# eloialonso/diamond

Hardware: AMD Instinct MI355X
Metric: imagined frames/sec (64x64, 3 denoise steps, batch 256) (higher is better)
Workload: dtype f32 via split-f16 MFMA (world-model convs (3x3 stride 1 / 2, 1x1): fp32 operands split into 2 x fp16 pieces, 3 x v_mfma_f32_*_f16 per product, fp32 accumulate (fp32-class, 22-bit operands); attention core, linears: exact fp32 v_mfma_f32_16x16x4_f32; actor-critic encoder forward, dgrad and weight-gra

## Files before the change

### diamond_amd/csrc/dmd_linear.hip

```cpp
#include "dmd_common.h"

#define LIN_DEPTH 4

__device__ __forceinline__ f32x4 lin_frag(const float* rowp, size_t ks, int k, int K) {
  f32x4 v;
#pragma unroll
  for (int t = 0; t < 4; ++t) {
    const int kk = k + t;
    const float x = rowp[(size_t)(kk < K ? kk : K - 1) * ks];
    v[t] = kk < K ? x : 0.f;
  }
  return v;
}

template <bool SPLITK, bool TRANS>
__device__ __forceinline__ void linear_mfma_body(const dmd_linear_params& p) {
  __shared__ f32x4 part[SPLITK ? 3 : 1][4][64];
  const int lane = threadIdx.x & 63, wave = threadIdx.x >> 6;
  const int i = lane & 15, kg = lane >> 4;
  const int m0 = SPLITK ? blockIdx.x * 32 : blockIdx.x * 64 + (wave >> 1) * 32;
  const int n0 = SPLITK ? blockIdx.y * 32 : blockIdx.y * 64 + (wave & 1) * 32;
  const int Kp = TRANS ? (p.K + 15) & ~15 : p.K;
  const int kq = SPLITK ? Kp >> 2 : Kp;
  const int kbase = SPLITK ? wave * kq : 0;
  const int nsteps = kq >> 4;
  f32x4 acc[2][2];
#pragma unroll
  for (int a = 0; a < 2; ++a)
#pragma unroll
    for (int b = 0; b < 2; ++b) acc[a][b] = (f32x4){0.f, 0.f, 0.f, 0.f};

  const size_t a_rs = TRANS && p.trans_a ? 1 : (size_t)p.lda, a_ks = TRANS && p.trans_a ? (size_t)p.lda : 1;
  const size_t w_rs = TRANS && p.trans_w ? 1 : (size_t)p.ldw, w_ks = TRANS && p.trans_w ? (size_t)p.ldw : 1;
  const float* arow[2];
  const float* wrow[2];
#pragma unroll
  for (int b = 0; b < 2; ++b) {
    int m = m0 + 16 * b + i;
    m = m < p.M ? m : p.M - 1;
    int n = n0 + 16 * b + i;
    n = n < p.N ? n : p.N - 1;
    if (TRANS) {
      arow[b] = p.A + (size_t)m * a_rs;
      wrow[b] = p.W + (size_t)n * w_rs;
    } else {
      arow[b] = p.A + (size_t)m * p.lda + kbase + 4 * kg;
      wrow[b] = p.W + (size_t)n * p.ldw + kbase + 4 * kg;
    }
  }
  const int kl = kbase + 4 * kg;
  f32x4 af[LIN_DEPTH][2], wf[LIN_DEPTH][2];
#pragma unroll
  for (int d = 0; d < LIN_DEPTH; ++d) {
    const int ks = (d < nsteps ? d : nsteps - 1) * 16;
#pragma unroll
    for (int b = 0; b < 2; ++b) {
      if (TRANS) {
        af[d][b] = lin_frag(arow[b], a_ks, kl + ks, p.K);
        wf[d][b] = lin_frag(wrow[b], w_ks, kl + ks, p.K);
      } else {
        af[d][b] = *(const f32x4*)(arow[b] + ks);
        wf[d][b] = *(const f32x4*)(wrow[b] + ks);
      }
    }
  }
  for (int s0 = 0; s0 < nsteps; s0 += LIN_DEPTH) {
#pragma unroll
    for (int d = 0; d < LIN_DEPTH; ++d) {
      if (s0 + d < nsteps) {
#pragma unroll
        for (int nb = 0; nb < 2; ++nb)
#pragma unroll
          for (int mb = 0; mb < 2; ++mb)
#pragma unroll
            for (int t = 0; t < 4; ++t)
              acc[nb][mb] = __builtin_amdgcn_mfma_f32_16x16x4f32(wf[d][nb][t], af[d][mb][t], acc[nb][mb], 0, 0, 0);
        const int sn = s0 + d + LIN_DEPTH;
        const int ks = (sn < nsteps ? sn : nsteps - 1) * 16;
#pragma unroll
        for (int b = 0; b < 2; ++b) {
          if (TRANS) {
            af[d][b] = lin_frag(arow[b], a_ks, kl + ks, p.K);
            wf[d][b] = lin_frag(wrow[b], w_ks, kl + ks, p.K);
          } else {
            af[d][b] = *(const f32x4*)(arow[b] + ks);
            wf[d][b] = *(const f32x4*)(wrow[b] + ks);
          }
        }
      }
    }
  }
  if (SPLITK) {
    if (wave) {
#pragma unroll
      for (int nb = 0; nb < 2; ++nb)
#pragma unroll
        for (int mb = 0; mb < 2; ++mb) part[wave - 1][nb * 2 + mb][lane] = acc[nb][mb];
    }
    __syncthreads();
    if (wave) return;
#pragma unroll
    for (int w = 0; w < 3; ++w)
#pragma unroll
      for (int nb = 0; nb < 2; ++nb)
#pragma unroll
        for (int mb = 0; mb < 2; ++mb) acc[nb][mb] += part[w][nb * 2 + mb][lane];
  }
#pragma unroll
  for (int nb = 0; nb < 2; ++nb)
#pragma unroll
    for (int mb = 0; mb < 2; ++mb) {
      const int m = m0 + 16 * mb + i;
      const int n = n0 + 16 * nb + 4 * kg;
      if (m >= p.M) continue;
#pragma unroll
      for (int r = 0; r < 4; ++r) {
        if (n + r >= p.N) continue;
        float v = acc[nb][mb][r];
        if (p.bias) v += p.bias[n + r];
        float* c = p.C + (size_t)m * p.ldc + n + r;
        if (p.accumulate) v += *c;
        if (p.silu) v = dmd_silu(v);
        *c = v;
      }
    }
}

template <bool SPLITK>
__global__ __launch_bounds__(256) void linear_mfma_kernel(const dmd_linear_params p) {
  linear_mfma_body<SPLITK, false>(p);
}

template <bool SPLITK>
__global__ __launch_bounds__(256) void linear_mfma_t_kernel(const dmd_linear_params p) {
  linear_mfma_body<SPLITK, true>(p);
}

extern "C" int dmd_linear(const dmd_linear_params* p, dmd_stream_t stream) {
  DMD_CHECK_ARG(p && p->A && p->W && p->C, "linear: null");
  DMD_CHECK_ARG(p->M > 0 && p->N > 0 && p->K > 0, "linear: bad M/N/K %d %d %d", p->M, p->N, p->K);
  DMD_CHECK_ARG((p->trans_a | p->trans_w | 1) == 1, "linear: trans_a / trans_w are 0 or 1");
  const bool trans = p->trans_a || p->trans_w || p->K % 16 != 0 || p->lda % 4 != 0 || p->ldw % 4 != 0;
  const int Kp = (p->K + 15) / 16 * 16;
  const bool splitk = Kp >= 512 && Kp % 64 == 0;
  const dim3 grid = splitk ? dim3((p->M + 31) / 32, (p->N + 31) / 32) : dim3((p->M + 63) / 64, (p->N + 63) / 64);
  if (trans) {
    if (splitk)
      hipLaunchKernelGGL(linear_mfma_t_kernel<true>, grid, dim3(256), 0, (hipStream_t)stream, *p);
    else
      hipLaunchKernelGGL(linear_mfma_t_kernel<false>, grid, dim3(256), 0, (hipStream_t)stream, *p);
  } else if (splitk)
    hipLaunchKernelGGL(linear_mfma_kernel<true>, grid, dim3(256), 0, (hipStream_t)stream, *p);
  else
    hipLaunchKernelGGL(linear_mfma_kernel<false>, grid, dim3(256), 0, (hipStream_t)stream, *p);
  DMD_LAUNCH_CHECK();
  return 0;
}
```

### diamond_amd/native.py

```python
from __future__ import annotations

import ctypes as C
import os
from typing import Optional

import torch
from torch import Tensor

_HERE = os.path.dirname(os.path.abspath(__file__))
LIB_PATH = os.environ.get("DIAMOND_LIB", os.path.join(_HERE, "libdiamond_hip.so"))

PROLOGUE_NONE, PROLOGUE_NORM_SILU, PROLOGUE_NORM = 0, 1, 2
PRECISION_F32, PRECISION_F16X2 = 0, 1
GN_GROUP = 32


class NativeLibraryMissing(RuntimeError):
    pass


class Norm(C.Structure):
    _fields_ = [("stats", C.c_void_p), ("stat_tiles", C.c_int32), ("mul_plus_one", C.c_int32), ("mul", C.c_void_p),
                ("add", C.c_void_p), ("mul_stride", C.c_int64), ("add_stride", C.c_int64)]


class ConvSrc(C.Structure):
    _fields_ = [("x", C.c_void_p), ("C", C.c_int32), ("prologue", C.c_int32), ("norm", Norm)]


class ConvParams(C.Structure):
    _fields_ = [("N", C.c_int32), ("H", C.c_int32), ("W", C.c_int32), ("Cout", C.c_int32), ("CoutPad", C.c_int32),
                ("taps", C.c_int32), ("stride", C.c_int32), ("upsample", C.c_int32), ("nsrc", C.c_int32),
                ("src", ConvSrc * 2), ("w", C.c_void_p), ("bias", C.c_void_p), ("residual", C.c_void_p),
                ("residual_norm", Norm), ("out", C.c_void_p), ("out_nchw", C.c_int32), ("precision", C.c_int32),
                ("out_stats", C.c_void_p), ("w_f16", C.c_void_p), ("proj_nsrc", C.c_int32), ("proj_C", C.c_int32 * 2),
                ("proj_reserved", C.c_int32), ("proj_x", C.c_void_p * 2), ("proj_w_f16", C.c_void_p), ("proj_bias", C.c_void_p),
                ("valid_h", C.c_int32), ("valid_w", C.c_int32)]


class LinearParams(C.Structure):
    _fields_ = [("M", C.c_int32), ("N", C.c_int32), ("K", C.c_int32), ("A", C.c_void_p), ("lda", C.c_int64),
                ("W", C.c_void_p), ("ldw", C.c_int64), ("bias", C.c_void_p), ("C", C.c_void_p), ("ldc", C.c_int64),
                ("accumulate", C.c_int32), ("silu", C.c_int32), ("trans_a", C.c_int32), ("trans_w", C.c_int32)]


class GnBwdParams(C.Structure):
    _fields_ = [("N", C.c_int32), ("HW", C.c_int32), ("C", C.c_int32), ("identity_activation", C.c_int32), ("x", C.c_void_p),
                ("norm", Norm), ("da", C.c_void_p), ("dskip", C.c_void_p), ("dx", C.c_void_p), ("workspace", C.c_void_p),
                ("dmul", C.c_void_p), ("dadd", C.c_void_p), ("W", C.c_int32), ("valid_h", C.c_int32), ("valid_w", C.c_int32),
                ("reserved", C.c_int32)]


class WgradParams(C.Structure):
    _fields_ = [("N", C.c_int32), ("H", C.c_int32), ("W", C.c_int32), ("Cout", C.c_int32), ("taps", C.c_int32),
                ("cin_real", C.c_int32), ("src", ConvSrc), ("dy", C.c_void_p), ("workspace", C.c_void_p), ("dw", C.c_void_p),
                ("dbias", C.c_void_p), ("precision", C.c_int32), ("valid_h", C.c_int32), ("valid_w", C.c_int32), ("defer_reduce", C.c_int32)]


class WgradReduceJob(C.Structure):
    _fields_ = [("partials", C.c_void_p), ("dw", C.c_void_p), ("dbias", C.c_void_p), ("num_wg", C.c_int32), ("NB", C.c_int32),
                ("NCO", C.c_int32), ("NCI", C.c_int32), ("taps", C.c_int32), ("cin_real", C.c_int32), ("ld_cin", C.c_int32),
                ("c0", C.c_int32), ("scale", C.c_void_p), ("kind", C.c_int32), ("reserved", C.c_int32)]


REDUCE_WGRAD, REDUCE_COLSUM = 0, 1


class DgradInputParams(C.Structure):
    _fields_ = [("N", C.c_int32), ("H", C.c_int32), ("W", C.c_int32), ("valid_h", C.c_int32), ("valid_w", C.c_int32), ("Cout", C.c_int32),
                ("cin", C.c_int32), ("c_split", C.c_int32), ("dy", C.c_void_p), ("w", C.c_void_p), ("dx_a", C.c_void_p), ("dx_b", C.c_void_p),
                ("scale_a", C.c_void_p), ("stride_a", C.c_int32), ("scale_b", C.c_float), ("post", C.c_void_p), ("swap_scales", C.c_int32),
                ("reserved", C.c_int32)]


class PackJob(C.Structure):
    _fields_ = [("src", C.c_void_p), ("dst", C.c_void_p), ("Cout", C.c_int32), ("Cin", C.c_int32), ("k", C.c_int32),
                ("kind", C.c_int32), ("transposed", C.c_int32), ("c0", C.c_int32), ("c1", C.c_int32), ("CoutPad", C.c_int32),
                ("CinPad", C.c_int32), ("reserved", C.c_int32)]


PACK_F32, PACK_F16X2, PACK_BIAS = 0, 1, 2


class ChecksumJob(C.Structure):
    _fields_ = [("src", C.c_void_p), ("words", C.c_int64)]


CHECKSUM_PARTS = 8


class PoolRound(C.Structure):
    _fields_ = [("frames", C.c_void_p), ("pad", C.c_void_p), ("act", C.c_void_p), ("hx", C.c_void_p), ("cx", C.c_void_p),
                ("is_f32", C.c_int32), ("rows", C.c_int32)]


class ResetSlotsParams(C.Structure):
    _fields_ = [("B", C.c_int32), ("K", C.c_int32), ("T", C.c_int32), ("head", C.c_int32), ("per_frame", C.c_int64),
                ("hd", C.c_int32), ("reserved", C.c_int32), ("pool", PoolRound * 2), ("pool_base", C.c_int64), ("num_dead", C.c_void_p),
                ("slot_row", C.c_void_p), ("row_slot", C.c_void_p), ("next_obs", C.c_void_p), ("ctx", C.c_void_p),
                ("act_ring", C.c_void_p), ("hx", C.c_void_p), ("cx", C.c_void_p), ("enc_in", C.c_void_p)]


class SegmentGatherParams(C.Structure):
    _fields_ = [("B", C.c_int32), ("T", C.c_int32), ("per_frame", C.c_int64), ("flag_size", C.c_int32), ("put_back_final", C.c_int32),
                ("frames", C.c_void_p), ("act", C.c_void_p), ("rew", C.c_void_p), ("end", C.c_void_p), ("trunc", C.c_void_p),
                ("finals", C.c_void_p), ("seg", C.c_void_p), ("out_obs", C.c_void_p), ("out_act", C.c_void_p), ("out_rew", C.c_void_p),
                ("out_end", C.c_void_p), ("out_trunc", C.c_void_p), ("out_mask", C.c_void_p), ("out_final", C.c_void_p)]


class OpenLoopParams(C.Structure):
    _fields_ = [("B", C.c_int32), ("T", C.c_int32), ("per_frame", C.c_int64), ("step", C.c_int32), ("head", C.c_int32),
                ("teacher_forced", C.c_int32), ("reserved", C.c_int32), ("frames", C.c_void_p), ("act", C.c_void_p), ("rew", C.c_void_p),
                ("end", C.c_void_p), ("finals", C.c_void_p), ("seg", C.c_void_p), ("pred", C.c_void_p), ("ctx_obs", C.c_void_p),
                ("ctx_act", C.c_void_p), ("metrics", C.c_void_p), ("out_rew", C.c_void_p), ("out_end", C.c_void_p),
                ("out_valid", C.c_void_p), ("out_levels", C.c_void_p)]


SSIM_TAPS = 11


class SsimParams(C.Structure):
    _fields_ = [("N", C.c_int32), ("C", C.c_int32), ("H", C.c_int32), ("W", C.c_int32), ("a_f32", C.c_void_p), ("a_u8", C.c_void_p),
                ("b_f32", C.c_void_p), ("b_u8", C.c_void_p), ("frames", C.c_void_p), ("finals", C.c_void_p), ("end", C.c_void_p),
                ("seg", C.c_void_p), ("T", C.c_int32), ("step", C.c_int32), ("win", C.c_double * SSIM_TAPS), ("c1", C.c_double),
                ("c2", C.c_double), ("workspace", C.c_void_p), ("out", C.c_void_p)]


CHAIN_MAX_BLOCKS = 8


class ChainBlock(C.Structure):
    _fields_ = [("skip_slot", C.c_int32), ("save_slot", C.c_int32), ("film1_mul", C.c_int32 * 2), ("film1_add", C.c_int32 * 2),
                ("film2_mul", C.c_int32), ("film2_add", C.c_int32), ("has_attn", C.c_int32), ("reserved", C.c_int32),
                ("w1", C.c_void_p), ("w2", C.c_void_p), ("wproj", C.c_void_p), ("b1", C.c_void_p), ("b2", C.c_void_p),
                ("bproj", C.c_void_p), ("gn_gamma", C.c_void_p), ("gn_beta", C.c_void_p), ("wq", C.c_void_p), ("wk", C.c_void_p),
                ("wv", C.c_void_p), ("wo", C.c_void_p), ("bqkv", C.c_void_p), ("bo", C.c_void_p)]


class LowresChainParams(C.Structure):
    _fields_ = [("N", C.c_int32), ("nblocks", C.c_int32), ("input_save_slot", C.c_int32), ("reserved", C.c_int32),
                ("x", C.c_void_p), ("out", C.c_void_p), ("table", C.c_void_p), ("table_stride", C.c_int64),
                ("blocks", ChainBlock * CHAIN_MAX_BLOCKS)]


EXPORTS = (
    "dmd_conv2d", "dmd_conv2d_kernel_name", "dmd_conv2d_naive", "dmd_conv_stat_tiles", "dmd_pack_conv_weight", "dmd_conv2d_f16x2_eligible",
    "dmd_conv1x1_stream_eligible", "dmd_conv2d_proj_eligible", "dmd_pack_jobs", "dmd_checksums",
    "dmd_pack_conv_weight_f16x2", "dmd_linear", "dmd_attention", "dmd_attention_valid", "dmd_attention_f32", "dmd_attention_f16x2", "dmd_attention_bwd", "dmd_attention_bwd_valid",
    "dmd_attention_bwd_mfma", "dmd_attention_bwd_workspace_floats",
    "dmd_edm_pack_input", "dmd_cond_embed", "dmd_edm_denoised", "dmd_euler_step", "dmd_heun_step", "dmd_quantize_u8", "dmd_reset_state",
    "dmd_dequant_gather", "dmd_segment_gather", "dmd_openloop_step", "dmd_frame_ssim", "dmd_ssim_workspace_doubles", "dmd_resolve_deaths", "dmd_reset_slots", "dmd_merge_slots", "dmd_merge_slots_bwd", "dmd_nchw_to_nhwc",
    "dmd_nhwc_to_nchw", "dmd_gn_stats", "dmd_gn_stats_valid", "dmd_maxpool2", "dmd_lstm_pointwise", "dmd_lstm_pointwise_bwd", "dmd_lambda_returns", "dmd_categorical_sample", "dmd_rew_end_loss",
    "dmd_maxpool2_bwd", "dmd_gn_bwd_workspace_bytes", "dmd_gn_silu_bwd", "dmd_wgrad_workspace_floats", "dmd_conv2d_wgrad", "dmd_wgrad_job", "dmd_wgrad_reduce_jobs",
    "dmd_conv2d_dgrad_input", "dmd_lowres_chain", "dmd_lowres_chain32", "dmd_last_error", "dmd_abi_version", "dmd_reload_env",
)

LAUNCHERS = frozenset(n for n in EXPORTS if n not in (
    "dmd_conv2d_kernel_name", "dmd_conv_stat_tiles", "dmd_conv2d_f16x2_eligible", "dmd_conv1x1_stream_eligible",
    "dmd_conv2d_proj_eligible", "dmd_attention_bwd_workspace_floats", "dmd_gn_bwd_workspace_bytes", "dmd_wgrad_workspace_floats", "dmd_wgrad_job", "dmd_ssim_workspace_doubles", "dmd_last_error",
    "dmd_abi_version", "dmd_reload_env"))


class LaunchProfiler:

    def __init__(self) -> None:
        self.records = []
        self._pending = None

    def annotate(self, key: str, flops: float, nbytes: float) -> None:
        self._pending = (key, flops, nbytes)

    def call(self, name: str, fn, args):
        key, flops, nbytes = self._pending or (name, 0.0, 0.0)
        self._pending = None
        e0, e1 = torch.cuda.Event(enable_timing=True), torch.cuda.Event(enable_timing=True)
        e0.record()
        rc = fn(*args)
        e1.record()
        self.records.append((key, flops, nbytes, e0, e1))
        return rc

    def summary(self):
        torch.cuda.synchronize()
        out = {}
        for key, flops, nbytes, e0, e1 in self.records:
            d = out.setdefault(key, {"launches": 0, "ms": 0.0, "flops": 0.0, "bytes": 0.0})
            d["launches"] += 1
            d["ms"] += e0.elapsed_time(e1)
            d["flops"] += flops
            d["bytes"] += nbytes
        return out


PROFILER: Optional[LaunchProfiler] = None


class _Lib:

    def __init__(self, cdll: C.CDLL) -> None:
        self._cdll = cdll

    def __getattr__(self, name: str):
        fn = getattr(self._cdll, name)
        if name not in LAUNCHERS:
            return fn

        def launch(*args):
            prof = PROFILER
            return fn(*args) if prof is None else prof.call(name, fn, args)

        return launch


def declare_signatures(L: C.CDLL) -> None:
    L.dmd_last_error.restype = C.c_char_p
    L.dmd_reload_env.restype = None
    for name in EXPORTS:
        getattr(L, name)
    L.dmd_conv2d.argtypes = [C.POINTER(ConvParams), C.c_void_p]
    L.dmd_conv2d_naive.argtypes = [C.POINTER(ConvParams), C.c_void_p]
    L.dmd_conv2d_kernel_name.argtypes = [C.POINTER(ConvParams), C.c_char_p, C.c_int]
    L.dmd_linear.argtypes = [C.POINTER(LinearParams), C.c_void_p]
    L.dmd_pack_conv_weight.argtypes = [C.c_void_p, C.c_void_p, C.c_int, C.c_int, C.c_int, C.c_int, C.c_int, C.c_void_p]
    L.dmd_pack_conv_weight_f16x2.argtypes = [C.c_void_p, C.c_void_p, C.c_int, C.c_int, C.c_int, C.c_int, C.c_void_p]
    L.dmd_conv2d_f16x2_eligible.argtypes = [C.POINTER(ConvParams)]
    L.dmd_conv1x1_stream_eligible.argtypes = [C.POINTER(ConvParams)]
    L.dmd_conv2d_proj_eligible.argtypes = [C.POINTER(ConvParams)]
    L.dmd_pack_jobs.argtypes = [C.c_void_p, C.c_int, C.c_int64, C.c_void_p]
    L.dmd_checksums.argtypes = [C.c_void_p, C.c_int, C.c_void_p, C.c_void_p]
    L.dmd_attention.argtypes = [C.c_void_p, C.c_void_p, C.c_int, C.c_int, C.c_int, C.c_int, C.c_void_p]
    L.dmd_attention_valid.argtypes = [C.c_void_p, C.c_void_p, C.c_int, C.c_int, C.c_int, C.c_int, C.c_int, C.c_int, C.c_int, C.c_void_p]
    L.dmd_attention_f32.argtypes = list(L.dmd_attention_valid.argtypes)
    L.dmd_attention_f16x2.argtypes = list(L.dmd_attention_valid.argtypes)
    L.dmd_attention_bwd.argtypes = [C.c_void_p, C.c_void_p, C.c_void_p, C.c_void_p, C.c_void_p, C.c_int, C.c_int, C.c_int,
                                    C.c_int, C.c_void_p]
    L.dmd_attention_bwd_valid.argtypes = [C.c_void_p, C.c_void_p, C.c_void_p, C.c_void_p, C.c_void_p, C.c_int, C.c_int, C.c_int,
                                          C.c_int, C.c_int, C.c_int, C.c_int, C.c_void_p]
    L.dmd_attention_bwd_mfma.argtypes = list(L.dmd_attention_bwd_valid.argtypes)
    L.dmd_attention_bwd_workspace_floats.argtypes = [C.c_int, C.c_int, C.c_int]
    L.dmd_attention_bwd_workspace_floats.restype = C.c_int64
    L.dmd_edm_pack_input.argtypes = [C.c_void_p, C.c_void_p, C.c_void_p, C.c_int, C.c_float, C.c_void_p, C.c_int, C.c_int,
                                     C.c_int, C.c_int, C.c_int, C.c_int, C.c_int, C.c_int, C.c_void_p]
    L.dmd_cond_embed.argtypes = [C.c_void_p, C.c_int, C.c_void_p, C.c_void_p, C.c_void_p, C.c_void_p, C.c_int,
                                 C.c_int, C.c_int, C.c_int, C.c_int, C.c_int, C.c_void_p]
    L.dmd_heun_step.argtypes = [C.c_void_p, C.c_void_p, C.c_void_p, C.c_void_p, C.c_float, C.c_float, C.c_float,
                                C.c_void_p, C.c_int64, C.c_void_p]
    L.dmd_quantize_u8.argtypes = [C.c_void_p, C.c_void_p, C.c_void_p, C.c_int64, C.c_void_p]
    L.dmd_dequant_gather.argtypes = [C.c_void_p, C.c_void_p, C.c_void_p, C.c_void_p, C.c_int, C.c_int, C.c_int64,
                                     C.c_int, C.c_void_p]
    L.dmd_segment_gather.argtypes = [C.POINTER(SegmentGatherParams), C.c_void_p]
    L.dmd_openloop_step.argtypes = [C.POINTER(OpenLoopParams), C.c_void_p]
    L.dmd_frame_ssim.argtypes = [C.POINTER(SsimParams), C.c_void_p]
    L.dmd_ssim_workspace_doubles.argtypes = [C.c_int, C.c_int, C.c_int, C.c_int]
    L.dmd_ssim_workspace_doubles.restype = C.c_int64
    L.dmd_reset_state.argtypes = [C.c_void_p, C.c_void_p, C.c_int, C.c_void_p, C.c_void_p, C.c_int, C.c_int, C.c_void_p, C.c_void_p,
                                  C.c_void_p, C.c_void_p, C.c_int, C.c_void_p, C.c_void_p]
    L.dmd_resolve_deaths.argtypes = [C.c_void_p, C.c_void_p, C.c_int, C.c_void_p, C.c_void_p, C.c_int, C.c_int, C.c_void_p, C.c_void_p,
                                     C.c_void_p, C.c_void_p]
    L.dmd_reset_slots.argtypes = [C.POINTER(ResetSlotsParams), C.c_void_p]
    L.dmd_merge_slots.argtypes = [C.c_void_p, C.c_void_p, C.c_void_p, C.c_void_p, C.c_int, C.c_int, C.c_void_p]
    L.dmd_merge_slots_bwd.argtypes = [C.c_void_p, C.c_void_p, C.c_void_p, C.c_void_p, C.c_void_p, C.c_int, C.c_int, C.c_int, C.c_void_p]
    L.dmd_edm_denoised.argtypes = [C.c_void_p, C.c_void_p, C.c_void_p, C.c_int, C.c_void_p, C.c_int, C.c_int64,
                                   C.c_void_p]
    L.dmd_euler_step.argtypes = [C.c_void_p, C.c_void_p, C.c_float, C.c_float, C.c_void_p, C.c_int64, C.c_void_p]
    L.dmd_nchw_to_nhwc.argtypes = [C.c_void_p, C.c_void_p, C.c_int, C.c_int, C.c_int, C.c_int, C.c_int, C.c_void_p]
    L.dmd_nhwc_to_nchw.argtypes = [C.c_void_p, C.c_void_p, C.c_int, C.c_int, C.c_int, C.c_int, C.c_int, C.c_void_p]
    L.dmd_gn_stats.argtypes = [C.c_void_p, C.c_void_p, C.c_int, C.c_int, C.c_int, C.c_void_p]
    L.dmd_gn_stats_valid.argtypes = [C.c_void_p, C.c_void_p, C.c_int, C.c_int, C.c_int, C.c_int, C.c_int, C.c_int, C.c_void_p]
    L.dmd_maxpool2.argtypes = [C.c_void_p, C.c_void_p, C.c_void_p, C.c_void_p, C.c_int, C.c_int, C.c_int, C.c_int,
                               C.c_void_p]
    L.dmd_lstm_pointwise.argtypes = [C.c_void_p, C.c_void_p, C.c_void_p, C.c_void_p, C.c_int, C.c_int, C.c_void_p]
    L.dmd_lstm_pointwise_bwd.argtypes = [C.c_void_p, C.c_void_p, C.c_void_p, C.c_void_p, C.c_void_p, C.c_void_p, C.c_void_p,
                                         C.c_int, C.c_int, C.c_void_p]
    L.dmd_lambda_returns.argtypes = [C.c_void_p, C.c_void_p, C.c_void_p, C.c_void_p, C.c_void_p, C.c_int, C.c_int, C.c_float, C.c_float,
                                     C.c_float, C.c_void_p]
    L.dmd_categorical_sample.argtypes = [C.c_void_p, C.c_void_p, C.c_void_p, C.c_int, C.c_int, C.c_void_p]
    L.dmd_rew_end_loss.argtypes = [C.c_void_p, C.c_void_p, C.c_void_p, C.c_void_p, C.c_void_p, C.c_void_p, C.c_void_p, C.c_int, C.c_void_p]
    L.dmd_conv_stat_tiles.argtypes = [C.c_int, C.c_int]
    L.dmd_maxpool2_bwd.argtypes = [C.c_void_p, C.c_void_p, C.c_void_p, C.c_int, C.c_int, C.c_int, C.c_int, C.c_void_p]
    L.dmd_gn_bwd_workspace_bytes.argtypes = [C.c_int, C.c_int, C.c_int]
    L.dmd_gn_bwd_workspace_bytes.restype = C.c_int64
    L.dmd_gn_silu_bwd.argtypes = [C.POINTER(GnBwdParams), C.c_void_p]
    L.dmd_wgrad_workspace_floats.argtypes = [C.POINTER(WgradParams)]
    L.dmd_wgrad_workspace_floats.restype = C.c_int64
    L.dmd_conv2d_wgrad.argtypes = [C.POINTER(WgradParams), C.c_void_p]
    L.dmd_wgrad_job.argtypes = [C.POINTER(WgradParams), C.POINTER(WgradReduceJob)]
    L.dmd_wgrad_reduce_jobs.argtypes = [C.c_void_p, C.c_int, C.c_void_p]
    L.dmd_conv2d_dgrad_input.argtypes = [C.POINTER(DgradInputParams), C.c_void_p]
    L.dmd_lowres_chain.argtypes = [C.POINTER(LowresChainParams), C.c_void_p]
    L.dmd_lowres_chain32.argtypes = [C.POINTER(LowresChainParams), C.c_void_p]


_lib: Optional[_Lib] = None


def lib() -> _Lib:
    global _lib
    if _lib is None:
        if not os.path.exists(LIB_PATH):
            raise NativeLibraryMissing(
                f"{LIB_PATH} not found: build it with `python -c 'import __graft_entry__ as g; g.build()'` "
                "(diamond_amd has no CPU/PyTorch fallback for its kernels)")
        L = C.CDLL(LIB_PATH)
        if hasattr(L, "dmd_simt_host_build"):
            raise NativeLibraryMissing(
                f"{LIB_PATH} is the SIMT-interpreter build of the kernels (tests/simt, test infrastructure): "
                "diamond_amd runs on libdiamond_hip.so only, there is no CPU path")
        declare_signatures(L)
        _lib = _Lib(L)
    return _lib


def check(rc: int, what: str) -> None:
    if rc != 0:
        raise RuntimeError(f"{what} failed (rc={rc}): {lib().dmd_last_error().decode()}")


def stream() -> int:
    return torch.cuda.current_stream().cuda_stream


def check_current_device(dev: torch.device) -> None:
    if dev.type == "cuda" and dev.index is not None and dev.index != torch.cuda.current_device():
        raise RuntimeError(f"diamond_amd: the module lives on {dev} but the current device is cuda:{torch.cuda.current_device()}: "
                           f"call torch.cuda.set_device({dev.index}) (or wrap the call in torch.cuda.device({dev.index}))")


def require_gpu(t: Tensor) -> None:
    if not t.is_cuda:
        raise RuntimeError("diamond_amd kernels need GPU tensors (there is no CPU path)")


def ptr(t: Optional[Tensor]) -> Optional[int]:
    if t is None:
        return None
    require_gpu(t)
    return t.data_ptr()


def fptr(t: Optional[Tensor]) -> Optional[int]:
    if t is not None:
        assert t.dtype == torch.float32 and t.is_contiguous(), (t.dtype, t.shape, t.stride())
    return ptr(t)


def conv_stat_tiles(h: int, w: int) -> int:
    return (h // 8) * (w // (8 if w % 16 else 16))


def cout_pad(cout: int) -> int:
    return (cout + 15) // 16 * 16


def make_norm(stats: Optional[Tensor] = None, stat_tiles: int = 0, mul: Optional[Tensor] = None,
              add: Optional[Tensor] = None, mul_stride: int = 0, add_stride: int = 0, plus_one: bool = False) -> Norm:
    n = Norm()
    n.stats = ptr(stats)
    n.stat_tiles = stat_tiles
    n.mul_plus_one = int(plus_one)
    n.mul = ptr(mul)
    n.add = ptr(add)
    n.mul_stride = mul_stride
    n.add_stride = add_stride
    return n


def pack_conv_weight(w_oihw: Tensor, cout_padded: Optional[int] = None) -> Tensor:
    cout, cin, k, _ = w_oihw.shape
    cp = cout_padded or cout_pad(cout)
    cinp = (cin + 15) // 16 * 16
    w = w_oihw.detach().contiguous().float()
    out = torch.empty(cinp // 16 * k * k * cp * 16, device=w.device, dtype=torch.float32)
    check(lib().dmd_pack_conv_weight(fptr(w), fptr(out), cout, cin, k, cp, cinp, stream()), "dmd_pack_conv_weight")
    return out


def pack_conv_weight_f16x2(w_oihw: Tensor) -> Tensor:
    cout, cin, k, _ = w_oihw.shape
    assert cout in (32, 64) and k in (1, 3), (cout, k)
    cinp = (cin + 15) // 16 * 16
    w = w_oihw.detach().contiguous().float()
    out = torch.empty(cinp // 16 * k * k * 2 * cout * 16, device=w.device, dtype=torch.float16)
    check(lib().dmd_pack_conv_weight_f16x2(fptr(w), ptr(out), cout, cin, k, cinp, stream()), "dmd_pack_conv_weight_f16x2")
    return out


def pad_vector(v: Optional[Tensor], n: int) -> Optional[Tensor]:
    if v is None:
        return None
    out = torch.zeros(n, device=v.device, dtype=torch.float32)
    out[: v.numel()] = v.detach().float()
    return out


def linear(a: Tensor, w: Tensor, bias: Optional[Tensor], out: Tensor, accumulate: bool = False, silu: bool = False) -> Tensor:
    p = LinearParams()
    p.M, p.K = a.shape
    p.N = w.shape[0]
    assert w.shape[1] == p.K and out.shape == (p.M, p.N), (a.shape, w.shape, out.shape)
    assert out.stride(1) == 1 and a.dtype == w.dtype == out.dtype == torch.float32

    def operand(t: Tensor):
        if t.stride(1) == 1 or t.shape[1] == 1:
            return 0, t.stride(0)
        assert t.stride(0) == 1 or t.shape[0] == 1, f"linear: operand strides {t.stride()}: neither storage order"
        return 1, t.stride(1)

    p.trans_a, p.lda = operand(a)
    p.trans_w, p.ldw = operand(w)
    p.A, p.W = ptr(a), ptr(w)
    p.bias = ptr(bias)
    p.C, p.ldc = ptr(out), out.stride(0)
    p.accumulate, p.silu = int(accumulate), int(silu)
    if PROFILER is not None:
        PROFILER.annotate(f"linear_mfma_kernel<{'true' if (p.K + 15) // 16 * 16 >= 512 else 'false'}>", 2.0 * p.M * p.N * p.K,
                          4.0 * (p.M * p.K + p.N * p.K + p.M * p.N))
    check(lib().dmd_linear(C.byref(p), stream()), "dmd_linear")
    return out
```

### include/diamond_hip.h

```cpp
#ifndef DIAMOND_HIP_H
#define DIAMOND_HIP_H

#include <stdint.h>

#ifdef __cplusplus
extern "C" {
#endif

typedef void* dmd_stream_t;

#define DMD_PROLOGUE_NONE 0
#define DMD_PROLOGUE_NORM_SILU 1
#define DMD_PROLOGUE_NORM 2

#define DMD_GN_GROUP 32

typedef struct dmd_norm {
  const double* stats;
  int32_t stat_tiles;
  int32_t mul_plus_one;
  const float* mul;
  const float* add;
  int64_t mul_stride;
  int64_t add_stride;
} dmd_norm;

typedef struct dmd_conv_src {
  const float* x;
  int32_t C;
  int32_t prologue;
  dmd_norm norm;
} dmd_conv_src;

typedef struct dmd_conv_params {
  int32_t N, H, W;
  int32_t Cout;
  int32_t CoutPad;
  int32_t taps;
  int32_t stride;
  int32_t upsample;
  int32_t nsrc;
  dmd_conv_src src[2];
  const float* w;
  const float* bias;
  const float* residual;
  dmd_norm residual_norm;
  float* out;
  int32_t out_nchw;
  int32_t precision;
  double* out_stats;
  const void* w_f16;
  int32_t proj_nsrc;
  int32_t proj_C[2];
  int32_t proj_reserved;
  const float* proj_x[2];
  const void* proj_w_f16;
  const float* proj_bias;
  int32_t valid_h, valid_w;
} dmd_conv_params;

#define DMD_PRECISION_F32 0
#define DMD_PRECISION_F16X2 1
int dmd_conv2d_f16x2_eligible(const dmd_conv_params* p);
int dmd_conv2d_proj_eligible(const dmd_conv_params* p);
int dmd_conv1x1_stream_eligible(const dmd_conv_params* p);
int dmd_pack_conv_weight_f16x2(const float* oihw, void* packed, int Cout, int Cin, int k, int CinPad, dmd_stream_t stream);

#define DMD_PACK_F32 0
#define DMD_PACK_F16X2 1
#define DMD_PACK_BIAS 2
typedef struct dmd_pack_job {
  const float* src;
  void* dst;
  int32_t Cout, Cin, k;
  int32_t kind, transposed, c0, c1;
  int32_t CoutPad, CinPad;
  int32_t reserved;
} dmd_pack_job;
int dmd_pack_jobs(const dmd_pack_job* jobs_device, int njobs, int64_t max_elems, dmd_stream_t stream);

#define DMD_CHECKSUM_PARTS 8
typedef struct dmd_checksum_job {
  const void* src;
  int64_t words;
} dmd_checksum_job;
int dmd_checksums(const dmd_checksum_job* jobs_device, int njobs, long long* out_device, dmd_stream_t stream);

int dmd_conv2d(const dmd_conv_params* p, dmd_stream_t stream);
int dmd_conv2d_kernel_name(const dmd_conv_params* p, char* buf, int buf_len);
int dmd_conv_stat_tiles(int H, int W);
int dmd_pack_conv_weight(const float* oihw, float* packed, int Cout, int Cin, int k, int CoutPad, int CinPad,
                         dmd_stream_t stream);

int dmd_conv2d_naive(const dmd_conv_params* p, dmd_stream_t stream);

typedef struct dmd_linear_params {
  int32_t M, N, K;
  const float* A; int64_t lda;
  const float* W; int64_t ldw;
  const float* bias;
  float* C; int64_t ldc;
  int32_t accumulate;
  int32_t silu;
  int32_t trans_a, trans_w;
} dmd_linear_params;
int dmd_linear(const dmd_linear_params* p, dmd_stream_t stream);

int dmd_attention(const float* qkv, float* out, int N, int T, int C, int head_dim, dmd_stream_t stream);
int dmd_attention_valid(const float* qkv, float* out, int N, int H, int W, int valid_h, int valid_w, int C, int head_dim,
                        dmd_stream_t stream);
int dmd_attention_f32(const float* qkv, float* out, int N, int H, int W, int valid_h, int valid_w, int C, int head_dim,
                      dmd_stream_t stream);
int dmd_attention_f16x2(const float* qkv, float* out, int N, int H, int W, int valid_h, int valid_w, int C, int head_dim,
                        dmd_stream_t stream);
int64_t dmd_attention_bwd_workspace_floats(int N, int T, int C);
int dmd_attention_bwd(const float* qkv, const float* y, const float* dy, float* dqkv, float* workspace, int N, int T, int C,
                      int head_dim, dmd_stream_t stream);
int dmd_attention_bwd_valid(const float* qkv, const float* y, const float* dy, float* dqkv, float* workspace, int N, int H, int W,
                            int valid_h, int valid_w, int C, int head_dim, dmd_stream_t stream);
int dmd_attention_bwd_mfma(const float* qkv, const float* y, const float* dy, float* dqkv, float* workspace, int N, int H, int W,
                           int valid_h, int valid_w, int C, int head_dim, dmd_stream_t stream);

#define DMD_CHAIN_MAX_BLOCKS 8
typedef struct dmd_chain_block {
  int32_t skip_slot;
  int32_t save_slot;
  int32_t film1_mul[2];
  int32_t film1_add[2];
  int32_t film2_mul, film2_add;
  int32_t has_attn, reserved;
  const void* w1;
  const void* w2;
  const void* wproj;
  const float* b1;
  const float* b2;
  const float* bproj;
  const float* gn_gamma;
  const float* gn_beta;
  const void* wq;
  const void* wk;
  const void* wv;
  const void* wo;
  const float* bqkv;
  const float* bo;
} dmd_chain_block;

typedef struct dmd_lowres_chain_params {
  int32_t N;
  int32_t nblocks;
  int32_t input_save_slot;
  int32_t reserved;
  const float* x;
  float* out;
  const float* table;
  int64_t table_stride;
  dmd_chain_block blocks[DMD_CHAIN_MAX_BLOCKS];
} dmd_lowres_chain_params;
int dmd_lowres_chain(const dmd_lowres_chain_params* p, dmd_stream_t stream);
int dmd_lowres_chain32(const dmd_lowres_chain_params* p, dmd_stream_t stream);


int dmd_edm_pack_input(const float* x, const float* obs, const float* cond, int cond_stride, float sigma_data,
                       float* out_nhwc, int N, int Cx, int Cobs, int H, int W, int CPad, int T, int head,
                       dmd_stream_t stream);
int dmd_cond_embed(const float* cond, int cond_stride, const float* fourier_w ,
                   const int64_t* act , const float* act_emb , float* out , int N,
                   int half, int T, int E, int act_head, int A, dmd_stream_t stream);
int dmd_edm_denoised(const float* x, const float* model_out, const float* cond, int cond_stride,
                     float* denoised, int N, int64_t per_sample, dmd_stream_t stream);
int dmd_euler_step(const float* x, const float* denoised, float sigma_hat, float dt, float* x_out, int64_t n,
                   dmd_stream_t stream);
int dmd_heun_step(const float* x, const float* denoised, const float* x_2, const float* denoised_2, float sigma_hat,
                  float sigma_next, float dt, float* x_out, int64_t n, dmd_stream_t stream);

int dmd_quantize_u8(const float* x, uint8_t* q, int* off_grid, int64_t n, dmd_stream_t stream);
int dmd_dequant_gather(const uint8_t* pool, const int64_t* idx, const int64_t* rows, float* dst, int M, int T,
                       int64_t per_frame, int head, dmd_stream_t stream);
int dmd_reset_state(const int64_t* idx, const int64_t* rows, int count, const int64_t* pool_act, int64_t* act_ring, int T, int head,
                    const float* pool_hx, const float* pool_cx, float* hx, float* cx, int hd, int64_t* ep_len, dmd_stream_t stream);

int dmd_resolve_deaths(const int64_t* end, int64_t* ep_len, int horizon, int64_t* trunc, uint8_t* dead, int B, int K,
                       int64_t* slot_row, int32_t* row_slot, int32_t* report, dmd_stream_t stream);

typedef struct dmd_pool_round {
  const void* frames;
  const uint8_t* pad;
  const int64_t* act;
  const float* hx;
  const float* cx;
  int32_t is_f32, rows;
} dmd_pool_round;
typedef struct dmd_reset_slots_params {
  int32_t B, K, T, head;
  int64_t per_frame;
  int32_t hd, reserved;
  dmd_pool_round pool[2];
  int64_t pool_base;
  const int32_t* num_dead;
  const int64_t* slot_row;
  const int32_t* row_slot;
  const float* next_obs;
  float* ctx;
  int64_t* act_ring;
  float* hx;
  float* cx;
  float* enc_in;
} dmd_reset_slots_params;
int dmd_reset_slots(const dmd_reset_slots_params* p, dmd_stream_t stream);

typedef struct dmd_segment_gather_params {
  int32_t B, T;
  int64_t per_frame;
  int32_t flag_size;
  int32_t put_back_final;
  const uint8_t* frames;
  const int64_t* act;
  const float* rew;
  const uint8_t* end;
  const uint8_t* trunc;
  const uint8_t* finals;
  const int64_t* seg;
  float* out_obs;
  int64_t* out_act;
  float* out_rew;
  void* out_end;
  void* out_trunc;
  uint8_t* out_mask;
  float* out_final;
} dmd_segment_gather_params;
int dmd_segment_gather(const dmd_segment_gather_params* p, dmd_stream_t stream);

typedef struct dmd_openloop_params {
  int32_t B, T;
  int64_t per_frame;
  int32_t step, head;
  int32_t teacher_forced;
  int32_t reserved;
  const uint8_t* frames;
  const int64_t* act;
  const float* rew;
  const uint8_t* end;
  const uint8_t* finals;
  const int64_t* seg;
  const float* pred;
  float* ctx_obs;
  int64_t* ctx_act;
  int64_t* metrics;
  float* out_rew;
  uint8_t* out_end;
  uint8_t* out_valid;
  uint8_t* out_levels;
} dmd_openloop_params;
int dmd_openloop_step(const dmd_openloop_params* p, dmd_stream_t stream);

#define DMD_SSIM_TAPS 11
typedef struct dmd_ssim_params {
  int32_t N, C, H, W;
  const float* a_f32;
  const uint8_t* a_u8;
  const float* b_f32;
  const uint8_t* b_u8;
  const uint8_t* frames;
  const uint8_t* finals;
  const uint8_t* end;
  const int64_t* seg;
  int32_t T, step;
  double win[DMD_SSIM_TAPS];
  double c1, c2;
  double* workspace;
  double* out;
} dmd_ssim_params;
int64_t dmd_ssim_workspace_doubles(int N, int C, int H, int W);
int dmd_frame_ssim(const dmd_ssim_params* p, dmd_stream_t stream);

int dmd_merge_slots(const float* base, const float* slots, const int32_t* row_slot, float* out, int B, int D, dmd_stream_t stream);
int dmd_merge_slots_bwd(const float* d_out, const int32_t* row_slot, const int64_t* slot_row, float* d_base, float* d_slots, int B, int K,
                        int D, dmd_stream_t stream);

int dmd_nchw_to_nhwc(const float* in, float* out, int N, int C, int H, int W, int CPad, dmd_stream_t stream);
int dmd_nhwc_to_nchw(const float* in, float* out, int N, int C, int H, int W, int CPad, dmd_stream_t stream);

int dmd_gn_stats(const float* x, double* stats, int N, int HW, int C, dmd_stream_t stream);
int dmd_gn_stats_valid(const float* x, double* stats, int N, int H, int W, int valid_h, int valid_w, int C, dmd_stream_t stream);

int dmd_maxpool2(const float* x, float* out, uint8_t* argmax, double* out_stats, int N, int H, int W, int C,
                 dmd_stream_t stream);

int dmd_lstm_pointwise(const float* gates, const float* c_prev, float* h, float* c, int N, int Hd,
                       dmd_stream_t stream);

int dmd_lstm_pointwise_bwd(const float* gates, const float* c_prev, const float* c_new, const float* dh, const float* dc,
                           float* dgates, float* dc_prev, int N, int Hd, dmd_stream_t stream);
int dmd_lambda_returns(const float* rew, const int64_t* end, const int64_t* trunc, const float* val_bootstrap, float* ret, int B, int T,
                       float gamma, float one_minus_lambda, float lambda, dmd_stream_t stream);

int dmd_categorical_sample(const float* logits, const float* expo, int64_t* out, int N, int A, dmd_stream_t stream);

int dmd_rew_end_loss(const float* logits, const float* rew, const int64_t* end, const uint8_t* mask, float* losses, float* dlogits,
                     int64_t* counts, int R, dmd_stream_t stream);


int dmd_maxpool2_bwd(const float* dpooled, const uint8_t* argmax, float* dx, int N, int H, int W, int C,
                     dmd_stream_t stream);

typedef struct dmd_gn_bwd_params {
  int32_t N, HW, C;
  int32_t identity_activation;
  const float* x;
  dmd_norm norm;
  const float* da;
  const float* dskip;
  float* dx;
  void* workspace;
  float* dmul;
  float* dadd;
  int32_t W, valid_h, valid_w, reserved;
} dmd_gn_bwd_params;
int64_t dmd_gn_bwd_workspace_bytes(int N, int HW, int C);
int dmd_gn_silu_bwd(const dmd_gn_bwd_params* p, dmd_stream_t stream);

typedef struct dmd_wgrad_params {
  int32_t N, H, W;
  int32_t Cout;
  int32_t taps;
  int32_t cin_real;
  dmd_conv_src src;
  const float* dy;
  float* workspace;
  float* dw;
  float* dbias;
  int32_t precision;
  int32_t valid_h, valid_w;
  int32_t defer_reduce;
} dmd_wgrad_params;
int64_t dmd_wgrad_workspace_floats(const dmd_wgrad_params* p);
int dmd_conv2d_wgrad(const dmd_wgrad_params* p, dmd_stream_t stream);

typedef struct dmd_wgrad_reduce_job {
  const float* partials;
  float* dw;
  float* dbias;
  int32_t num_wg, NB, NCO, NCI, taps, cin_real;
  int32_t ld_cin, c0;
  const float* scale;
  int32_t kind, reserved;
} dmd_wgrad_reduce_job;
#define DMD_REDUCE_WGRAD 0
#define DMD_REDUCE_COLSUM 1
int dmd_wgrad_job(const dmd_wgrad_params* p, dmd_wgrad_reduce_job* job);
int dmd_wgrad_reduce_jobs(const dmd_wgrad_reduce_job* jobs, int njobs, dmd_stream_t stream);

typedef struct dmd_dgrad_input_params {
  int32_t N, H, W;
  int32_t valid_h, valid_w;
  int32_t Cout;
  int32_t cin, c_split;
  const float* dy;
  const float* w;
  float* dx_a;
  float* dx_b;
  const float* scale_a;
  int32_t stride_a;
  float scale_b;
  const float* post;
  int32_t swap_scales;
  int32_t reserved;
} dmd_dgrad_input_params;
int dmd_conv2d_dgrad_input(const dmd_dgrad_input_params* p, dmd_stream_t stream);

const char* dmd_last_error(void);
int dmd_abi_version(void);
void dmd_reload_env(void);

#ifdef __cplusplus
}
#endif
#endif
```

Before: 13070.

## Stage linear GEMM operands through swizzled LDS with adaptive tile size selection

Replaces the non-transposed fp32 MFMA linear kernel with one that cooperatively loads A and W chunks into double-buffered, XOR-swizzled LDS, prefetching several chunks ahead in registers. Tiles are reused across waves instead of each wave loading its own fragments from global memory. A host heuristic picks smaller tiles (down to 16x16 with in-block split-K) when the grid would have fewer than two workgroups per CU, and a 1D grid is remapped per XCD. The old kernel is kept behind an environment switch. The trade-off is extra barriers and LDS traffic, and linears are likely a small share of the frame pipeline.

```diff
diff --git a/diamond_amd/csrc/dmd_linear.hip b/diamond_amd/csrc/dmd_linear.hip
--- a/diamond_amd/csrc/dmd_linear.hip
+++ b/diamond_amd/csrc/dmd_linear.hip
@@ -1,4 +1,6 @@
 #include "dmd_common.h"
+
+#include <type_traits>
 
 #define LIN_DEPTH 4
 
@@ -126,17 +128,214 @@
     }
 }
 
+namespace linear_v1 {
 template <bool SPLITK>
 __global__ __launch_bounds__(256) void linear_mfma_kernel(const dmd_linear_params p) {
   linear_mfma_body<SPLITK, false>(p);
 }
+}
+
+#define LIN_AHEAD 3
+#define LIN_LDS_SLOTS 4096
+
+template <bool SPLITK, bool WQ, int MB, int NB, int KCS, int PF>
+__device__ __forceinline__ void linear_tile_body(const dmd_linear_params& p, f32x4* lds) {
+  constexpr int TM = (WQ ? 16 : 32) * MB, TN = (WQ ? 16 : 32) * NB, ROWS = TM + TN;
+  constexpr int SLOTS = 4 * KCS;
+  constexpr int LPT = ROWS * SLOTS / 256;
+  constexpr int RSTEP = 256 / SLOTS;
+  constexpr int SPQ = SPLITK ? KCS / 4 : KCS;
+  constexpr int NACC = SPLITK && !WQ ? 4 : 1;
+  static_assert(2 * ROWS * SLOTS <= LIN_LDS_SLOTS && 256 % SLOTS == 0 && TM % RSTEP == 0 && KCS % 4 == 0 && (SPLITK || !WQ), "linear tile");
+  const int tid = threadIdx.x, lane = tid & 63, wave = tid >> 6;
+  const int i = lane & 15, kg = lane >> 4;
+
+  const int tiles_m = (p.M + TM - 1) / TM;
+  const int nwg = gridDim.x, b = blockIdx.x;
+  const int q8 = nwg >> 3, r8 = nwg & 7, x8 = b & 7;
+  const int tile = (x8 < r8 ? x8 * (q8 + 1) : r8 * (q8 + 1) + (x8 - r8) * q8) + (b >> 3);
+  const int m0 = (tile % tiles_m) * TM, n0 = (tile / tiles_m) * TN;
+
+  const int nsteps = SPLITK ? p.K >> 6 : p.K >> 4;
+  const int kq = SPLITK ? p.K >> 2 : 0;
+  const int nchunks = (nsteps + SPQ - 1) / SPQ;
+
+  const int fslot = tid % SLOTS, fj = fslot >> 2;
+  const int fset = fj / SPQ, fu = fj % SPQ;
+  const int r0 = tid / SLOTS;
+  const float* frow[LPT];
+#pragma unroll
+  for (int l = 0; l < LPT; ++l) {
+    const int r = r0 + l * RSTEP;
+    if (r < TM) {
+      int m = m0 + r;
+      m = m < p.M ? m : p.M - 1;
+      frow[l] = p.A + (size_t)m * p.lda + fset * kq + 4 * (fslot & 3);
+    } else {
+      int n = n0 + r - TM;
+      n = n < p.N ? n : p.N - 1;
+      frow[l] = p.W + (size_t)n * p.ldw + fset * kq + 4 * (fslot & 3);
+    }
+  }
+  f32x4 st[PF][LPT];
+  auto fetch = [&](f32x4* dst, int c) {
+    const int sn = c * SPQ + fu;
+    const int s = sn < nsteps ? sn : nsteps - 1;
+#pragma unroll
+    for (int l = 0; l < LPT; ++l) dst[l] = *(const f32x4*)(frow[l] + s * 16);
+  };
+#pragma unroll
+  for (int u = 0; u < PF; ++u) fetch(st[u], u);
+
+  f32x4 acc[NACC][NB][MB];
+#pragma unroll
+  for (int a = 0; a < NACC; ++a)
+#pragma unroll
+    for (int nb = 0; nb < NB; ++nb)
+#pragma unroll
+      for (int mb = 0; mb < MB; ++mb) acc[a][nb][mb] = (f32x4){0.f, 0.f, 0.f, 0.f};
+
+  const int wm = WQ ? 0 : (wave >> 1) * 16 * MB, wn = WQ ? 0 : (wave & 1) * 16 * NB;
+  const int arow = wm + i;
+  const int wrow = TM + wn + i;
+  auto steps = [&](const f32x4* buf, int left, auto whole) {
+#pragma unroll
+    for (int jj = 0; jj < (WQ ? SPQ : KCS); ++jj) {
+      const int j = WQ ? wave * SPQ + jj : jj;
+      if (decltype(whole)::value || jj % SPQ < left) {
+        f32x4 af[MB], wf[NB];
+#pragma unroll
+        for (int mb = 0; mb < MB; ++mb) af[mb] = buf[(arow + 16 * mb) * SLOTS + ((4 * j + kg) ^ i)];
+#pragma unroll
+        for (int nb = 0; nb < NB; ++nb) wf[nb] = buf[(wrow + 16 * nb) * SLOTS + ((4 * j + kg) ^ i)];
+#pragma unroll
+        for (int nb = 0; nb < NB; ++nb)
+#pragma unroll
+          for (int mb = 0; mb < MB; ++mb)
+#pragma unroll
+            for (int t = 0; t < 4; ++t)
+              acc[NACC > 1 ? jj / SPQ : 0][nb][mb] =
+                  __builtin_amdgcn_mfma_f32_16x16x4f32(wf[nb][t], af[mb][t], acc[NACC > 1 ? jj / SPQ : 0][nb][mb], 0, 0, 0);
+      }
+    }
+  };
+  for (int c0 = 0; c0 < nchunks; c0 += PF) {
+#pragma unroll
+    for (int u = 0; u < PF; ++u) {
+      const int c = c0 + u;
+      if (c < nchunks) {
+        f32x4* buf = lds + (c & 1) * (ROWS * SLOTS);
+#pragma unroll
+        for (int l = 0; l < LPT; ++l) {
+          const int r = r0 + l * RSTEP;
+          buf[r * SLOTS + (fslot ^ (r & 15))] = st[u][l];
+        }
+        __syncthreads();
+        if (c + PF < nchunks) fetch(st[u], c + PF);
+        const int left = nsteps - c * SPQ;
+        if (left >= SPQ)
+          steps(buf, left, std::true_type{});
+        else
+          steps(buf, left, std::false_type{});
+      }
+    }
+  }
+  if (WQ) {
+    __syncthreads();
+    if (wave) {
+#pragma unroll
+      for (int nb = 0; nb < NB; ++nb)
+#pragma unroll
+        for (int mb = 0; mb < MB; ++mb) lds[((wave - 1) * NB * MB + nb * MB + mb) * 64 + lane] = acc[0][nb][mb];
+    }
+    __syncthreads();
+    if (wave) return;
+#pragma unroll
+    for (int w = 0; w < 3; ++w)
+#pragma unroll
+      for (int nb = 0; nb < NB; ++nb)
+#pragma unroll
+        for (int mb = 0; mb < MB; ++mb) acc[0][nb][mb] += lds[(w * NB * MB + nb * MB + mb) * 64 + lane];
+  } else if (SPLITK) {
+#pragma unroll
+    for (int w = 1; w < NACC; ++w)
+#pragma unroll
+      for (int nb = 0; nb < NB; ++nb)
+#pragma unroll
+        for (int mb = 0; mb < MB; ++mb) acc[0][nb][mb] += acc[w][nb][mb];
+  }
+#pragma unroll
+  for (int nb = 0; nb < NB; ++nb)
+#pragma unroll
+    for (int mb = 0; mb < MB; ++mb) {
+      const int m = m0 + wm + 16 * mb + i;
+      const int n = n0 + wn + 16 * nb + 4 * kg;
+      if (m >= p.M) continue;
+#pragma unroll
+      for (int r = 0; r < 4; ++r) {
+        if (n + r >= p.N) continue;
+        float v = acc[0][nb][mb][r];
+        if (p.bias) v += p.bias[n + r];
+        float* c = p.C + (size_t)m * p.ldc + n + r;
+        if (p.accumulate) v += *c;
+        if (p.silu) v = dmd_silu(v);
+        *c = v;
+      }
+    }
+}
+
+struct LinTile {
+  int tm, tn;
+};
+static constexpr LinTile lin_tile(bool splitk, int tile) {
+  return tile >= 3 && splitk ? LinTile{16, 16} : tile >= 2 && splitk ? LinTile{16, 32} : tile >= 1 ? LinTile{32, 32} : splitk ? LinTile{32, 64} : LinTile{64, 64};
+}
+
+template <bool SPLITK>
+__global__ __launch_bounds__(256) void linear_mfma_kernel(const dmd_linear_params p, const int tile) {
+  __shared__ f32x4 lds[LIN_LDS_SLOTS];
+  if constexpr (SPLITK) {
+    if (tile >= 3) {
+      linear_tile_body<true, true, 1, 1, 16, LIN_AHEAD>(p, lds);
+      return;
+    }
+    if (tile == 2) {
+      linear_tile_body<true, true, 1, 2, 8, LIN_AHEAD>(p, lds);
+      return;
+    }
+  }
+  if (tile >= 1)
+    linear_tile_body<SPLITK, false, 1, 1, 8, LIN_AHEAD>(p, lds);
+  else
+    linear_tile_body<SPLITK, false, SPLITK ? 1 : 2, 2, 4, LIN_AHEAD>(p, lds);
+}
 
 template <bool SPLITK>
 __global__ __launch_bounds__(256) void linear_mfma_t_kernel(const dmd_linear_params p) {
   linear_mfma_body<SPLITK, true>(p);
 }
 
-extern "C" int dmd_linear(const dmd_linear_params* p, dmd_stream_t stream) {
+static int linear_pick_tile(const dmd_linear_params* p, bool splitk) {
+  static DmdEnvInt tile_env{"DIAMOND_LINEAR_TILE", -1};
+  const int last = splitk ? 3 : 1;
+  const int forced = tile_env.get();
+  if (forced >= 0) return forced < last ? forced : last;
+  static std::atomic<int> ncus[DMD_MAX_DEVICES];
+  int dev = 0;
+  if (hipGetDevice(&dev) != hipSuccess || dev < 0 || dev >= DMD_MAX_DEVICES) dev = 0;
+  int ncu = ncus[dev].load(std::memory_order_relaxed);
+  if (ncu <= 0) {
+    if (hipDeviceGetAttribute(&ncu, hipDeviceAttributeMultiprocessorCount, dev) != hipSuccess || ncu <= 0) ncu = 256;
+    ncus[dev].store(ncu, std::memory_order_relaxed);
+  }
+  for (int tile = 0; tile < last; ++tile) {
+    const LinTile t = lin_tile(splitk, tile);
+    if ((long long)((p->M + t.tm - 1) / t.tm) * ((p->N + t.tn - 1) / t.tn) >= 2 * ncu) return tile;
+  }
+  return last;
+}
+
+static int linear_launch(const dmd_linear_params* p, dmd_stream_t stream, bool v1) {
   DMD_CHECK_ARG(p && p->A && p->W && p->C, "linear: null");
   DMD_CHECK_ARG(p->M > 0 && p->N > 0 && p->K > 0, "linear: bad M/N/K %d %d %d", p->M, p->N, p->K);
   DMD_CHECK_ARG((p->trans_a | p->trans_w | 1) == 1, "linear: trans_a / trans_w are 0 or 1");
@@ -149,10 +348,25 @@
       hipLaunchKernelGGL(linear_mfma_t_kernel<true>, grid, dim3(256), 0, (hipStream_t)stream, *p);
     else
       hipLaunchKernelGGL(linear_mfma_t_kernel<false>, grid, dim3(256), 0, (hipStream_t)stream, *p);
-  } else if (splitk)
-    hipLaunchKernelGGL(linear_mfma_kernel<true>, grid, dim3(256), 0, (hipStream_t)stream, *p);
-  else
-    hipLaunchKernelGGL(linear_mfma_kernel<false>, grid, dim3(256), 0, (hipStream_t)stream, *p);
+  } else if (v1) {
+    if (splitk)
+      hipLaunchKernelGGL(linear_v1::linear_mfma_kernel<true>, grid, dim3(256), 0, (hipStream_t)stream, *p);
+    else
+      hipLaunchKernelGGL(linear_v1::linear_mfma_kernel<false>, grid, dim3(256), 0, (hipStream_t)stream, *p);
+  } else {
+    const int tile = linear_pick_tile(p, splitk);
+    const LinTile t = lin_tile(splitk, tile);
+    const long long tiles = (long long)((p->M + t.tm - 1) / t.tm) * ((p->N + t.tn - 1) / t.tn);
+    DMD_CHECK_ARG(tiles <= 0x7fffffffll, "linear: %lld tiles", tiles);
+    if (splitk)
+      hipLaunchKernelGGL(linear_mfma_kernel<true>, dim3((unsigned)tiles), dim3(256), 0, (hipStream_t)stream, *p, tile);
+    else
+      hipLaunchKernelGGL(linear_mfma_kernel<false>, dim3((unsigned)tiles), dim3(256), 0, (hipStream_t)stream, *p, tile);
+  }
   DMD_LAUNCH_CHECK();
   return 0;
 }
+
+extern "C" int dmd_linear(const dmd_linear_params* p, dmd_stream_t stream) { return linear_launch(p, stream, false); }
+
+extern "C" int dmd_linear_v1(const dmd_linear_params* p, dmd_stream_t stream) { return linear_launch(p, stream, true); }
diff --git a/diamond_amd/native.py b/diamond_amd/native.py
--- a/diamond_amd/native.py
+++ b/diamond_amd/native.py
@@ -146,7 +146,7 @@
 EXPORTS = (
     "dmd_conv2d", "dmd_conv2d_kernel_name", "dmd_conv2d_naive", "dmd_conv_stat_tiles", "dmd_pack_conv_weight", "dmd_conv2d_f16x2_eligible",
     "dmd_conv1x1_stream_eligible", "dmd_conv2d_proj_eligible", "dmd_pack_jobs", "dmd_checksums",
-    "dmd_pack_conv_weight_f16x2", "dmd_linear", "dmd_attention", "dmd_attention_valid", "dmd_attention_f32", "dmd_attention_f16x2", "dmd_attention_bwd", "dmd_attention_bwd_valid",
+    "dmd_pack_conv_weight_f16x2", "dmd_linear", "dmd_linear_v1", "dmd_attention", "dmd_attention_valid", "dmd_attention_f32", "dmd_attention_f16x2", "dmd_attention_bwd", "dmd_attention_bwd_valid",
     "dmd_attention_bwd_mfma", "dmd_attention_bwd_workspace_floats",
     "dmd_edm_pack_input", "dmd_cond_embed", "dmd_edm_denoised", "dmd_euler_step", "dmd_heun_step", "dmd_quantize_u8", "dmd_reset_state",
     "dmd_dequant_gather", "dmd_segment_gather", "dmd_openloop_step", "dmd_frame_ssim", "dmd_ssim_workspace_doubles", "dmd_resolve_deaths", "dmd_reset_slots", "dmd_merge_slots", "dmd_merge_slots_bwd", "dmd_nchw_to_nhwc",
@@ -221,6 +221,7 @@
     L.dmd_conv2d_naive.argtypes = [C.POINTER(ConvParams), C.c_void_p]
     L.dmd_conv2d_kernel_name.argtypes = [C.POINTER(ConvParams), C.c_char_p, C.c_int]
     L.dmd_linear.argtypes = [C.POINTER(LinearParams), C.c_void_p]
+    L.dmd_linear_v1.argtypes = [C.POINTER(LinearParams), C.c_void_p]
     L.dmd_pack_conv_weight.argtypes = [C.c_void_p, C.c_void_p, C.c_int, C.c_int, C.c_int, C.c_int, C.c_int, C.c_void_p]
     L.dmd_pack_conv_weight_f16x2.argtypes = [C.c_void_p, C.c_void_p, C.c_int, C.c_int, C.c_int, C.c_int, C.c_void_p]
     L.dmd_conv2d_f16x2_eligible.argtypes = [C.POINTER(ConvParams)]
@@ -415,5 +416,6 @@
     if PROFILER is not None:
         PROFILER.annotate(f"linear_mfma_kernel<{'true' if (p.K + 15) // 16 * 16 >= 512 else 'false'}>", 2.0 * p.M * p.N * p.K,
                           4.0 * (p.M * p.K + p.N * p.K + p.M * p.N))
-    check(lib().dmd_linear(C.byref(p), stream()), "dmd_linear")
+    entry = "dmd_linear_v1" if os.environ.get("DIAMOND_LINEAR") == "v1" else "dmd_linear"
+    check(getattr(lib(), entry)(C.byref(p), stream()), entry)
     return out
diff --git a/include/diamond_hip.h b/include/diamond_hip.h
--- a/include/diamond_hip.h
+++ b/include/diamond_hip.h
@@ -105,6 +105,7 @@
   int32_t trans_a, trans_w;
 } dmd_linear_params;
 int dmd_linear(const dmd_linear_params* p, dmd_stream_t stream);
+int dmd_linear_v1(const dmd_linear_params* p, dmd_stream_t stream);
 
 int dmd_attention(const float* qkv, float* out, int N, int T, int C, int head_dim, dmd_stream_t stream);
 int dmd_attention_valid(const float* qkv, float* out, int N, int H, int W, int valid_h, int valid_w, int C, int head_dim,
```

After: 13150 (median of 6 runs). Within noise of the previous version (+0.7%).
